# elcritch/figdraw

Measured on AMD Instinct MI355X. Metric: Mpixels/s composited @3840x2160, 300 SDF rects+shadows; % HBM roofline, higher is better.
Workload: dtype f32 (blur taps: u8 x f16 -> f32 MFMA); 1 GPU; S300@4K: renderlist_100 scene at 3840x2160, 300 shadowed SDF rects + full-frame and 360x240 2-pass Gaussian backdrop blur(18) (BASELINE.json configs[2]); draws=707, phases=3, blur_nodes=2, fragments=41088819, parallelism=single GPU, frames_in_flight_per_gpu=4, walk_pool_threads=7, walk_pool_threads_default=7

## Files before the change

### figdraw_amd/csrc/fdh_capi.cpp

```cpp
#include <string>

#include "fdh_context.h"
#include "fdh_damage.h"
#include "../../include/figdraw_hip_damage.h"
#include "../../include/figdraw_hip_pick.h"
#include "../../include/figdraw_hip_readback.h"
#include "../../include/figdraw_hip_stream.h"
#include "../../include/figdraw_hip_exact.h"
#include "../../include_glyphs/figdraw_hip_glyphs.h"
#include "../../include_glyphs/figdraw_hip_coverage.h"
#include "../../include_glyphs/figdraw_hip_cubic.h"

using fdh::Context;

namespace {
thread_local std::string g_last_error;

template <typename F>
int guard(F&& f) {
  try {
    f();
    return FDH_OK;
  } catch (const fdh::Error& e) {
    g_last_error = e.what();
// ... 12 lines not shown
}
}

extern "C" {

const char* fdh_last_error(void) { return g_last_error.c_str(); }
#if FDH_STATS
extern "C++" { namespace fdh { void debug_counters(unsigned long long out[128], bool reset); void debug_wave_times(unsigned long long* out); } }
__attribute__((visibility("default"))) int fdh_debug_wave_times(unsigned long long* out) { fdh::debug_wave_times(out); return 0; }
__attribute__((visibility("default"))) int fdh_debug_counters(unsigned long long out[128], int reset) { fdh::debug_counters(out, reset != 0); return 0; }
#endif
int fdh_saturated_core(const float rect[4], const float rx[4], const float ry[4], int mode, float factor, float spread,
                       const float shape[2], float aa, int out_px[4]) {
  return guard([&] { fdh::saturated_core_of(rect, rx, ry, mode, factor, spread, shape, aa, out_px); });
}
int fdh_blur_weight_fragments(float blur_radius, int vertical, float* dense, uint16_t* frag_bits, int* reach, int* k_steps) {
  return guard([&] {
    if (!dense || !frag_bits || !reach || !k_steps) throw fdh::Error(FDH_ERR_INVALID, "fdh_blur_weight_fragments: null pointer");
    fdh::blur_weight_fragments(blur_radius, vertical != 0, dense, frag_bits, reach, k_steps);
  });
}
const char* fdh_version(void) { return "figdraw_hip 0.1.0 (gfx950)"; }
int fdh_sizeof_fig(void) { return (int)sizeof(FdhFig); }
int fdh_sizeof_glyph(void) { return (int)sizeof(FdhGlyph); }
int fdh_sizeof_draw_op(void) { return (int)sizeof(FdhDrawOp); }
int fdh_sizeof_text_rect(void) { return (int)sizeof(FdhTextRect); }

int fdh_create(FdhContext** out, int atlas_size, float pixel_scale, int device, uint32_t flags) {
  return guard([&] {
    if (!out) throw fdh::Error(FDH_ERR_INVALID, "fdh_create: null out pointer");
// ... 325 lines not shown
```

### figdraw_amd/csrc/fdh_context.h

```cpp
#pragma once
#include <hip/hip_runtime.h>

#include <algorithm>
#include <atomic>
#include <chrono>
#include <condition_variable>
#include <cstdint>
#include <cstdlib>
#include <cstring>
#include <exception>
#include <memory>
#include <mutex>
#include <stdexcept>
#include <string>
#include <thread>
#include <unordered_map>
#include <vector>

#include "../../include/figdraw_hip.h"
#include "../../include/figdraw_hip_pick.h"
#include "../../include/figdraw_hip_readback.h"
#include "../../include/figdraw_hip_stream.h"
#include "fdh_kernels.h"
#include "fdh_plain.h"
#include "fdh_memory.h"
#include "fdh_frame.h"
#include "fdh_atlas.h"
#include "fdh_damage_host.h"
#include "fdh_retained.h"

namespace fdh {

struct RectMaskEntry { int kind; };
class Context;
struct SerialOnly {};

class Recorder {
 public:
  Recorder(Context* cx, bool is_main) : cx_(cx), is_main_(is_main) {}
  void save_transform();
  void restore_transform();
  void translate(float x, float y);
  void rotate(float a);
  void scale(float sx, float sy);
  void apply_transform(const float m[16]);
  bool transform_mirrors_y() const;
  void set_aa(float aa);
  float aa() const { return aa_; }
  void draw_rounded_rect_sdf(const float rect[4], const FdhColor colors[4], const float rx[4], const float ry[4], int mode,
                             float factor, float spread, const float shape[2], int fill_mode, FdhColor mid, FdhColor stop,
// ... 36 lines not shown
  BBox outer_union_{0, 0, 0, 0};
  int depth_now_ = 0;
  PhaseSum sum_;
  int64_t fragments_ = 0, culled_draws_ = 0;
  int phase_floor_ = 0;
  PickTag tag_{-1, -1};

 protected:
  DrawRec& next_rec();
  bool emit_quad(DrawRec& r, float x0, float y0, float x1, float y1, bool count_fragments);
  bool emit_quad_pts(DrawRec& r, const float vx[4], const float vy[4], bool count_fragments);
  struct QuadPx { float px[4], py[4]; BBox b; bool finite; };
  void quad_corners(const float vx[4], const float vy[4], QuadPx& q) const;
  bool emit_corners(DrawRec& r, const QuadPx& q, bool count_fragments);
  void push_rec(BBox b);
  void commit_bins(uint32_t idx);
  void link_share(uint32_t idx);
  bool bbox_visible(const BBox& b) const;
  struct EntryUV { const AtlasEntry* e; float S, x, y, w, h; };
  EntryUV entry_uv(int64_t key) const;
  struct PixelQuad { float x0, y0, x1, y1, w, h; };
  PixelQuad axis_lod(DrawRec& r, float S, float x0, float y0, float x1, float y1) const;
  void rect_entry();
  void white_texel_uv(DrawRec& r) const;
  void shrink_to_ink(const AtlasEntry& e, bool use_alpha, int level_t);
  friend class Context;
};

class Context : public Recorder {
 public:
// ... 277 lines not shown
};

template <typename Buf> void Context::reserve_quiet(Buf& buf, size_t n) {
  if (n <= buf.cap) return;
  drain();
  FDH_HIP(hipStreamSynchronize(stream_));
  buf.reserve(n);
}

void record_host_form(DrawRec& r);
void stripe_rows(int height, int world, int rank, int* y0, int* y1);
void comm_unique_id(uint8_t out[FDH_COMM_ID_BYTES]);
void blur_weight_fragments(float blur_radius, bool vertical, float* dense, uint16_t* frag_bits, int* reach, int* k_steps);
void saturated_core_of(const float rect[4], const float rx[4], const float ry[4], int mode, float factor, float spread,
                       const float shape[2], float aa, int out[4]);

}
```

### figdraw_amd/csrc/fdh_device.h

```cpp
#pragma once
#include <hip/hip_runtime.h>
#include <hip/hip_ext.h>
#include <stdint.h>
#include <algorithm>
#include <type_traits>

#include "fdh_kernels.h"

#include <cstddef>
#include <cstdlib>

namespace fdh {

#ifndef FDH_STATS
#define FDH_STATS 0
#endif
#ifndef FDH_TIMING
#define FDH_TIMING 0
#endif
#ifndef FDH_SPLIT_UNIFORM
#define FDH_SPLIT_UNIFORM 0
#endif
#if FDH_TIMING
#define FDH_NOW() clock64()
// ... 283 lines not shown
  x1 = x1 > kBin ? kBin : x1; y1 = y1 > kBin ? kBin : y1;
  const int r0 = y0 >> 3, r1 = (y1 + 7) >> 3;
  const uint32_t rows = ((1u << r1) - 1u) & ~((1u << r0) - 1u);
  return strips_of_rows(rows, x0 < kTileW, x1 > kTileW);
}

__device__ __forceinline__ uint32_t strip_mask_inside(int x0, int y0, int x1, int y1) {
  int r0 = (y0 + 7) >> 3, r1 = y1 >> 3;
  r0 = r0 < 0 ? 0 : r0; r0 = r0 > 8 ? 8 : r0; r1 = r1 > 8 ? 8 : r1;
  r1 = r1 < r0 ? r0 : r1;
  const uint32_t rows = ((1u << r1) - 1u) & ~((1u << r0) - 1u);
  const uint32_t m = strips_of_rows(rows, x0 <= 0 && x1 >= kTileW, x0 <= kTileW && x1 >= 2 * kTileW);
  return m & (0u - (uint32_t)(x1 > x0 && y1 > y0));
}

__device__ __forceinline__ bool bin_entry_head(const BinRec* __restrict__ binrec, int i, int x0, int y0, BinRec& r, uint32_t& word, uint32_t& strips) {
  {
    const uint2* __restrict__ src = reinterpret_cast<const uint2*>(binrec + i);
    uint2 q0 = src[0], q1 = src[1], q2 = src[2];
    asm volatile("" : "+v"(q0), "+v"(q1), "+v"(q2));
    r.box.x0 = (int16_t)(q0.x & 0xffffu); r.box.y0 = (int16_t)(q0.x >> 16); r.box.x1 = (int16_t)(q0.y & 0xffffu); r.box.y1 = (int16_t)(q0.y >> 16);
    r.ix0 = (int16_t)(q1.x & 0xffffu); r.iy0 = (int16_t)(q1.x >> 16); r.ix1 = (int16_t)(q1.y & 0xffffu); r.iy1 = (int16_t)(q1.y >> 16);
    r.flags = q2.x; r.pad = q2.y;
  }
  const BBox b = r.box;
  strips = strip_mask(b.x0 - x0, b.y0 - y0, b.x1 - x0, b.y1 - y0);
  word = (uint32_t)i | (r.flags & ~LE_INDEX);
  return b.x0 < x0 + kBin && b.x1 > x0 && b.y0 < y0 + kBin && b.y1 > y0;
}
__device__ __forceinline__ void bin_entry_tail(const BinRec& r, int x0, int y0, bool& hit, uint32_t& strips) {
  const uint32_t m_core = 0u - (uint32_t)((r.flags & BR_HAS_CORE) != 0u), m_removed = 0u - (uint32_t)((r.flags & BR_CORE_REMOVED) != 0u),
                 m_exact = 0u - (uint32_t)((r.flags & BR_BOX_EXACT) != 0u);
  const uint32_t core = strip_mask_inside(r.ix0 - x0, r.iy0 - y0, r.ix1 - x0, r.iy1 - y0) & strips & m_core;
  const uint32_t s1 = (strips & ~(core & m_removed)) | ((core & ~m_removed) << 16);
  const uint32_t m_gone = m_core & m_removed & (0u - (uint32_t)((s1 & 0xffffu) == 0u));
  const BBox b = r.box;
  const uint32_t inq = strip_mask_inside(b.x0 - x0, b.y0 - y0, b.x1 - x0, b.y1 - y0) & s1 & ~(s1 >> 16) & 0xffffu & m_core & m_exact & ~m_gone;
  strips = (s1 & ~inq) | (inq << 16);
  hit = hit && m_gone == 0u;
}

struct Frag {
  float u, v;
  F4 col;
  float fw_u, fw_v, lod;
  bool covered;
};

// ... 197 lines not shown
```

### figdraw_amd/csrc/fdh_record.cpp

```cpp
#include <algorithm>
#include <cmath>
#include <cstdio>
#include <cstring>

#include "fdh_context.h"
#include "fdh_host.h"

namespace fdh {

void Recorder::shrink_to_ink(const AtlasEntry& e, bool use_alpha, int level_t) {
  static const bool enabled = [] { const char* v = std::getenv("FDH_INK_BOUNDS"); return !v || std::atoi(v) != 0; }();
  if (!enabled || !e.has_ink || level_t < 0 || lane_->recs.empty()) return;
  DrawRec& r = lane_->recs.back();
  BBox& b = lane_->bins.back().box;
  if ((r.op_mode & F_GENERAL) || b.x1 <= b.x0 || b.y1 <= b.y0) return;
  const InkBox ib = (use_alpha ? e.ink_a : e.ink_rgb)[std::min(level_t / 16, kInkLevels - 1)];
  if (ib.x1 <= ib.x0 || ib.y1 <= ib.y0) { b = BBox{0, 0, 0, 0}; r.bx0 = r.by0 = r.bx1 = r.by1 = 0; return; }
  const double S = (double)cx_->atlas_.size();
  auto range = [&](double ua, double ut, double o, double inv, double lo_t, double hi_t, int& p0, int& p1) {
    const double A = (ut - ua) * inv * S, B = ua * S - 0.5 - A * o;
    if (!(std::fabs(A) > 1e-12)) return;
    double c0 = ((lo_t - 3.0) - B) / A, c1 = ((hi_t + 2.0) - B) / A;
    if (c0 > c1) std::swap(c0, c1);
    if (!(c0 > -1.0e6 && c1 < 1.0e6)) return;
// ... 80 lines not shown
void Recorder::apply_transform(const float m[16]) {
  { FDH_REC("apply_transform").fv(m, 16); }
  Aff n;
  n.a = m[0]; n.b = m[1]; n.c = m[4]; n.d = m[5]; n.tx = m[12]; n.ty = m[13];
  mat_ = aff_mul(mat_, n);
}
bool Recorder::transform_mirrors_y() const { return mat_.a * mat_.d - mat_.b * mat_.c < 0.0f; }

DrawRec& Recorder::next_rec() {
  DrawRec* r = lane_->recs.slot();
  std::memset(static_cast<void*>(r), 0, sizeof *r);
  return *r;
}
void Recorder::push_rec(BBox b) {
  BinRec* br = lane_->bins.slot();
  *br = BinRec{b, 0, 0, 0, 0, 0u, 0u};
  *lane_->boxes.slot() = 0x7f7f7f7fu;
  lane_->recs.n++;
  lane_->bins.n++;
  lane_->boxes.n++;
  if (cx_->pick_frame_) { *lane_->tags.slot() = tag_; lane_->tags.n++; }
}

uint32_t bin_box_of(const BBox& b, int shift) {
  if (bbox_empty(b)) return 0x7f7f7f7fu;
  return (uint32_t)(b.x0 >> shift) | ((uint32_t)(b.y0 >> shift) << 8) | ((127u - (uint32_t)((b.x1 - 1) >> shift)) << 16) | ((127u - (uint32_t)((b.y1 - 1) >> shift)) << 24);
}

static uint32_t binrec_flags(const DrawRec& r) {
  const uint32_t om = r.op_mode, op = (om >> 12) & 15u, mode = om & 255u, fill_mode = (om >> 9) & 7u;
  const bool atlas_mode = mode == 0u || (mode >= 13u && mode <= 16u);
// ... 148 lines not shown
    int run = 0;
    int* row = diff.data() + (size_t)y * dw;
    const int* above = y > ty0 ? row - dw : nullptr;
    for (int x = tx0; x < tx1; x++) {
      run += row[x];
      const int cell = run + (above ? above[x] : 0);
      row[x] = cell;
      mx = std::max(mx, cell);
    }
  }
  for (int y = ty0; y <= ty1; y++) std::fill(diff.begin() + (size_t)y * dw + tx0, diff.begin() + (size_t)y * dw + tx1 + 1, 0);
  touched = false;
  return mx;
}

static bool local_core(const DrawRec& r, double& xl, double& xr, double& yb, double& yt) {
  const uint32_t mode = r.op_mode & 255u, op = (r.op_mode >> 12) & 15u;
  const uint32_t fill_mode = (r.op_mode >> 9) & 7u;
  if (!(op == OP_DRAW || op == OP_MASK_PUSH) || !(r.aa > 0.0f)) return false;
  double e;
  if (op == OP_MASK_PUSH || mode == FDH_SDF_CLIP_AA || mode == FDH_SDF_BACKDROP_BLUR) e = 0.5 / r.aa;
  else if (mode == FDH_SDF_DROP_SHADOW) e = std::max(0.0, -(double)(fill_mode == 0u ? r.f1 : 0.0f));
  else if (mode == FDH_SDF_ANNULAR || mode == FDH_SDF_ANNULAR_AA) e = std::max(0.0, (double)r.f0) + 0.5 / r.aa;
  else if (mode == FDH_SDF_INSET_SHADOW && op == OP_DRAW) {
    const double sigma = std::max(0.5 * (double)r.f0, 0.5);
    e = std::max(0.0, 3.7 * sigma + (double)(fill_mode == 0u ? r.f1 : 0.0f));
  } else return false;
  const bool inset = mode == FDH_SDF_INSET_SHADOW;
  const double qhx = r.p0, qhy = r.p1, bx = inset ? qhx : (double)r.p2, by = inset ? qhy : (double)r.p3;
  if (!(qhx > 0.0 && qhy > 0.0 && bx > 0.0 && by > 0.0)) return false;
  double crx[4], cry[4];
  for (int k = 0; k < 4; k++) {
    const double sel = r.r[k];
    if (!(r.op_mode & F_ELLIP)) { crx[k] = cry[k] = std::max(sel, 0.0); continue; }
    if (sel < 0.0) { crx[k] = cry[k] = -sel - 1.0; continue; }
    const double pv = std::floor(sel + 0.5), hi = std::floor(pv / 4096.0);
    crx[k] = (pv - 4096.0 * hi) * bx / 4095.0;
    cry[k] = hi * by / 4095.0;
  }
  enum { TR = 0, BR = 1, TL = 2, BL = 3 };
  if (!(r.op_mode & F_ELLIP)) {
    const double k = 0.2929;
    auto rr = [&](int i) { return std::max(crx[i] - e, 0.0); };
    xr = (bx - e) - k * std::max(rr(TR), rr(BR));
    xl = -(bx - e) + k * std::max(rr(TL), rr(BL));
    yt = (by - e) - k * std::max(rr(TR), rr(TL));
    yb = -(by - e) + k * std::max(rr(BR), rr(BL));
  } else {
    const double hx0 = -(bx - e), hx1 = bx - e;
    const double hy1 = std::min(by - e, by - std::max(cry[TR], cry[TL])), hy0 = -std::min(by - e, by - std::max(cry[BR], cry[BL]));
    const double vy0 = -(by - e), vy1 = by - e;
    const double vx1 = std::min(bx - e, bx - std::max(crx[TR], crx[BR])), vx0 = -std::min(bx - e, bx - std::max(crx[TL], crx[BL]));
    const double ah = std::max(hx1 - hx0, 0.0) * std::max(hy1 - hy0, 0.0), av = std::max(vx1 - vx0, 0.0) * std::max(vy1 - vy0, 0.0);
    if (ah >= av) { xl = hx0; xr = hx1; yb = hy0; yt = hy1; } else { xl = vx0; xr = vx1; yb = vy0; yt = vy1; }
  }
  if (inset) { xl += r.p2; xr += r.p2; yb -= r.p3; yt -= r.p3; }
  return xr > xl && yt > yb;
}
static void set_saturated_core(DrawRec& r, float w_px, float h_px) {
  r.ix0 = r.iy0 = r.ix1 = r.iy1 = 0;
  double xl, xr, yb, yt;
  if (!local_core(r, xl, xr, yb, yt)) return;
  const double qhx = r.p0, qhy = r.p1;
#ifndef FDH_CORE_SLACK
#define FDH_CORE_SLACK (1.0 / 16.0)
#endif
  const double slack = FDH_CORE_SLACK;
  const double cxl = r.ox + w_px * (xl / (2.0 * qhx) + 0.5) + slack, cxr = r.ox + w_px * (xr / (2.0 * qhx) + 0.5) - slack;
  const double cyt = r.oy + h_px * (0.5 - yt / (2.0 * qhy)) + slack, cyb = r.oy + h_px * (0.5 - yb / (2.0 * qhy)) - slack;
  double ix0 = std::ceil(cxl - 0.5), ix1 = std::floor(cxr - 0.5) + 1.0, iy0 = std::ceil(cyt - 0.5), iy1 = std::floor(cyb - 0.5) + 1.0;
  ix0 = std::max(ix0, (double)r.ox); ix1 = std::min(ix1, (double)r.ox + w_px);
  iy0 = std::max(iy0, (double)r.oy); iy1 = std::min(iy1, (double)r.oy + h_px);
  auto c16 = [](double v) { return (int16_t)std::min(std::max(v, -32768.0), 32767.0); };
  if (!(ix1 > ix0 && iy1 > iy0)) return;
  r.ix0 = c16(ix0); r.iy0 = c16(iy0); r.ix1 = c16(ix1); r.iy1 = c16(iy1);
}

bool Recorder::emit_quad(DrawRec& r, float x0, float y0, float x1, float y1, bool count_fragments) {
  const float vx[4] = {x0, x1, x1, x0}, vy[4] = {y1, y1, y0, y0};
  return emit_quad_pts(r, vx, vy, count_fragments);
}

bool Recorder::rect_visible(const float rect[4], float pad) const {
  if (!(rect[2] > 0.0f) || !(rect[3] > 0.0f)) return false;
  const float vx[4] = {rect[0], rect[0] + rect[2], rect[0] + rect[2], rect[0]}, vy[4] = {rect[1] + rect[3], rect[1] + rect[3], rect[1], rect[1]};
  float minx = 0, maxx = 0, miny = 0, maxy = 0;
  for (int i = 0; i < 4; i++) {
    const float px = std::ceil(mat_.a * vx[i] + mat_.c * vy[i] + mat_.tx), py = std::ceil(mat_.b * vx[i] + mat_.d * vy[i] + mat_.ty);
    if (i == 0) { minx = maxx = px; miny = maxy = py; }
    else { minx = std::min(minx, px); maxx = std::max(maxx, px); miny = std::min(miny, py); maxy = std::max(maxy, py); }
// ... 22 lines not shown
  q.finite = minx > -lim && maxx < lim && miny > -lim && maxy < lim;
  if (!q.finite) return;
  const float W = (float)cx_->W_, H = (float)cx_->H_;
  q.b.x0 = (int16_t)clampf(minx, 0.0f, W); q.b.x1 = (int16_t)clampf(maxx, 0.0f, W);
  q.b.y0 = (int16_t)clampf(miny, 0.0f, H); q.b.y1 = (int16_t)clampf(maxy, 0.0f, H);
}
bool Recorder::emit_quad_pts(DrawRec& r, const float vx[4], const float vy[4], bool count_fragments) {
  QuadPx q;
  quad_corners(vx, vy, q);
  return emit_corners(r, q, count_fragments);
}
bool Recorder::emit_corners(DrawRec& r, const QuadPx& q, bool count_fragments) {
  const float* px = q.px;
  const float* py = q.py;
  BBox b = q.b;
  const bool cullable = ((r.op_mode >> 12) & 15u) == OP_DRAW && culling();
  const float fields[] = {r.p0, r.p1, r.p2, r.p3, r.f0, r.f1, r.r[0], r.r[1], r.r[2], r.r[3], r.aa, r.aux, r.aux2};
  bool params_finite = true;
  for (const float v : fields) params_finite = params_finite && std::isfinite(v);
  if (!q.finite || !params_finite) {
    if (cullable) { FDH_CULLED(); return false; }
    r.bx0 = r.by0 = r.bx1 = r.by1 = 0; push_rec(b); return true;
  }
  if (cullable && !bbox_visible(b)) { FDH_CULLED(); return false; }
  r.bx0 = b.x0; r.by0 = b.y0; r.bx1 = b.x1; r.by1 = b.y1;
  const bool aligned = px[3] == px[0] && px[2] == px[1] && py[3] == py[2] && py[0] == py[1] && px[1] > px[0] && py[0] > py[3];
  const bool bezier = (r.op_mode & 255u) >= 18u && (r.op_mode & 255u) <= 20u;
  if (aligned) {
    r.ox = px[3];
    r.oy = py[3];
    r.inv_w = 1.0f / (px[1] - px[0]);
    r.inv_h = 1.0f / (py[0] - py[3]);
    r.kx = 2.0f * r.p0 * r.inv_w;
    r.ky = 2.0f * r.p1 * r.inv_h;
    if (!bezier) set_saturated_core(r, px[1] - px[0], py[0] - py[3]);
  }
  if (!aligned || bezier) {
    QuadExt& q = *lane_->exts.slot();
    std::memset(static_cast<void*>(&q), 0, sizeof q);
    static const int TRI[2][3] = {{3, 0, 1}, {2, 3, 1}};
    const uint32_t mode = r.op_mode & 255u;
    const bool atlas_mode = mode == 0u || (mode >= 13u && mode <= 16u);
    const float uax = atlas_mode ? r.r[0] : 0.0f, uay = atlas_mode ? r.r[1] : 0.0f, utx = atlas_mode ? r.r[2] : 1.0f, uty = atlas_mode ? r.r[3] : 1.0f;
    const float vu[4] = {uax, utx, utx, uax}, vv[4] = {uty, uty, uay, uay};
    bool edge32 = true;
    const long long xm = 2LL * cx_->W_ + 129, ym = 2LL * cx_->H_ + 129;
    for (int t = 0; t < 2; t++) {
      long long X[3], Y[3];
      for (int k = 0; k < 3; k++) { X[k] = 2 * (long long)px[TRI[t][k]]; Y[k] = 2 * (long long)py[TRI[t][k]]; }
      long long area2 = (X[1] - X[0]) * (Y[2] - Y[0]) - (Y[1] - Y[0]) * (X[2] - X[0]);
// ... 25 lines not shown
        const double dv1 = vv[TRI[t][1]] - vv[TRI[t][0]], dv2 = vv[TRI[t][2]] - vv[TRI[t][0]];
        const double dudx = (du1 * e2y - du2 * e1y) / det, dudy = (du2 * e1x - du1 * e2x) / det;
        const double dvdx = (dv1 * e2y - dv2 * e1y) / det, dvdy = (dv2 * e1x - dv1 * e2x) / det;
        q.fw_u[t] = (float)(std::fabs(dudx) + std::fabs(dudy));
        q.fw_v[t] = (float)(std::fabs(dvdx) + std::fabs(dvdy));
        const double S = (double)cx_->atlas_.size();
        const double rho = std::max(std::sqrt(dudx * dudx + dvdx * dvdx), std::sqrt(dudy * dudy + dvdy * dvdy)) * S;
        q.lod[t] = rho > 0.0 ? (float)std::log2(rho) : 0.0f;
      } else {
        q.fw_u[t] = q.fw_v[t] = 1.0f;
      }
    }
    r.op_mode |= F_GENERAL;
    if (edge32) r.op_mode |= F_EDGE32;
    q.core[0] = q.core[1] = q.core[2] = q.core[3] = 0.0f;
    double xl, xr, yb, yt;
    if (edge32 && !atlas_mode && mode < 18u && ((r.op_mode >> 12) & 15u) == OP_DRAW && q.inv_sum[0] != 0.0f && q.inv_sum[1] != 0.0f && local_core(r, xl, xr, yb, yt)) {
      const double qhx = r.p0, qhy = r.p1;
      double sx = 0.0, sy = 0.0;
      for (int t = 0; t < 2; t++) {
        const QuadExt::Edge &E0 = q.e[t][0], &E1 = q.e[t][1], &E2 = q.e[t][2];
        const double is = (double)q.inv_sum[t];
        const double ua = t == 0 ? (double)E2.a : (double)E0.a + E2.a, ub = t == 0 ? (double)E2.b : (double)E0.b + E2.b, uc = t == 0 ? (double)E2.c : (double)E0.c + (double)E2.c;
        const double va = t == 0 ? (double)E1.a + E2.a : (double)E2.a, vb = t == 0 ? (double)E1.b + E2.b : (double)E2.b, vc = t == 0 ? (double)E1.c + (double)E2.c : (double)E2.c;
        const double kx = 2.0 * qhx * is, ky = -2.0 * qhy * is;
        const double m[6] = {kx * ua, kx * ub, kx * uc - qhx, ky * va, ky * vb, ky * vc + qhy};
        for (int k = 0; k < 6; k++) q.lm[t][k] = (float)m[k];
        sx = std::max(sx, 2.0 * (std::fabs(m[0]) + std::fabs(m[1])));
        sy = std::max(sy, 2.0 * (std::fabs(m[3]) + std::fabs(m[4])));
      }
#ifndef FDH_CORE_SLACK
#define FDH_CORE_SLACK (1.0 / 16.0)
// ... 61 lines not shown

void saturated_core_of(const float rect[4], const float rx[4], const float ry[4], int mode, float factor, float spread,
                       const float shape[2], float aa, int out[4]) {
  const FdhColor white{255, 255, 255, 255}, zero{0, 0, 0, 0};
  const FdhColor cols[4] = {white, white, white, white};
  DrawRec r;
  std::memset(static_cast<void*>(&r), 0, sizeof r);
  fill_sdf_rec(r, rect, cols, rx, ry, mode, factor, spread, shape, 0, zero, zero, 0.5f, aa);
  const float x0 = std::ceil(rect[0]), y0 = std::ceil(rect[1]), x1 = std::ceil(rect[0] + rect[2]), y1 = std::ceil(rect[1] + rect[3]);
  out[0] = out[1] = out[2] = out[3] = 0;
  if (!(x1 > x0 && y1 > y0)) return;
  r.ox = x0; r.oy = y0;
  r.inv_w = 1.0f / (x1 - x0); r.inv_h = 1.0f / (y1 - y0);
  set_saturated_core(r, x1 - x0, y1 - y0);
  out[0] = r.ix0; out[1] = r.iy0; out[2] = r.ix1; out[3] = r.iy1;
}

void Recorder::draw_rounded_rect_sdf(const float rect[4], const FdhColor colors[4], const float rx[4], const float ry[4], int mode,
                                    float factor, float spread, const float shape[2], int fill_mode, FdhColor mid, FdhColor stop,
                                    float mid_pos) {
  { FDH_REC("draw_rounded_rect_sdf").fv(rect, 4).cols(colors).fv(rx, 4).fv(ry, 4).i(mode).f(factor).f(spread).fv(shape, 2).i(fill_mode).col(mid).col(stop).f(mid_pos); }
  if (!cx_->frame_begun_) throw Error(FDH_ERR_INVALID, "ctx.beginFrame has not been called.");
  if (!(rect[2] > 0.0f) || !(rect[3] > 0.0f)) return;
  if (mode >= FDH_SDF_BEZIER_STROKE_AA) throw Error(FDH_ERR_INVALID, "bezier stroke modes go through drawQuadraticBezierSdf");
  QuadPx q;
  {
    const float x0 = rect[0], y0 = rect[1], x1 = rect[0] + rect[2], y1 = rect[1] + rect[3];
    const float vx[4] = {x0, x1, x1, x0}, vy[4] = {y1, y1, y0, y0};
    quad_corners(vx, vy, q);
  }
// ... 452 lines not shown
```

### figdraw_amd/csrc/fdh_types.h

```cpp
#pragma once
#include <stdint.h>

#ifndef FDH_MX_LO
#define FDH_MX_LO 0
#endif

namespace fdh {

constexpr int kTile = 8;
constexpr int kTileW = 4 * kTile;
constexpr int kTileH = kTile;
constexpr int kWavesPerWg = 4;
constexpr int kWgW = kTileW;
constexpr int kWgH = kTileH * kWavesPerWg;
constexpr int kBin = 64;
constexpr int kWgsPerBin = (kBin / kWgW) * (kBin / kWgH);
constexpr int kMaskDepth = 16;
constexpr int kDeepMinDefault = 24;
constexpr int kDeepMinInFlight = 40;
constexpr int kDeepStripMinDefault = 16;
constexpr int kMaxMips = 14;
constexpr int kMaxBlurTaps = 36;

enum : uint32_t { OP_DRAW = 0, OP_MASK_PUSH = 1, OP_MASK_POP = 2, OP_RMASK_BEGIN = 3, OP_RMASK_END = 4 };
// ... 30 lines not shown
struct alignas(16) QuadExt {
  struct Edge { int32_t a, b; int64_t c; };
  Edge e[2][3];
  float inv_sum[2];
  uint32_t own;
  float fw_u[2], fw_v[2];
  float lod[2];
  float _pad[3];
  float core[4];
  float lm[2][6];
};
static_assert(sizeof(QuadExt) == 208 && offsetof(QuadExt, core) == 144 && offsetof(QuadExt, lm) == 160, "QuadExt: 208 bytes, core at 144, lm at 160");

struct alignas(8) BBox { int16_t x0, y0, x1, y1; };

struct alignas(8) BinRec { BBox box; int16_t ix0, iy0, ix1, iy1; uint32_t flags; uint32_t pad; };
static_assert(sizeof(BinRec) == 24, "BinRec must be 24 bytes");
constexpr uint32_t BR_HAS_CORE = 1u, BR_CORE_REMOVED = 2u;
constexpr uint32_t BR_GENERAL = 4u;
constexpr uint32_t BR_CURVE = 8u;
constexpr uint32_t BR_BOX_EXACT = 16u;
constexpr uint32_t LE_PLAIN = 1u << 31;
constexpr uint32_t LE_OPAQUE = 1u << 30;
constexpr int LE_PATH_SHIFT = 26;
constexpr uint32_t LE_SHARE = 1u << 25;
constexpr uint32_t LE_INDEX = LE_SHARE - 1u;

constexpr int kMaxBlurReach = 66;
constexpr int kBlurPad = 15;
struct BlurTaps {
  int n;
  int reach;
// ... 23 lines not shown
```

### figdraw_amd/csrc/k_bin_upload.hip

```cpp
#include "fdh_device.h"

namespace fdh {
__device__ __forceinline__ bool binbox_hits(uint32_t q, uint32_t U) { return ((U - q) & 0x80808080u) == 0x80808080u; }
template <bool kRefine>
__device__ __forceinline__ void bin_entry(const BinParams& P, int i, int x0, int y0, bool& hit, uint32_t& word, uint32_t& strips) {
  BinRec r;
  if (!bin_entry_head(P.binrec, i, x0, y0, r, word, strips)) { hit = false; return; }
  if (kRefine && (r.flags & BR_CURVE)) {
    const uint4* __restrict__ d4 = reinterpret_cast<const uint4*>(P.draws + i);
    const uint4 q0 = d4[0], q1 = d4[1], q2 = d4[2], q3 = d4[3], q5 = d4[5];
    const float ox = __uint_as_float(q0.z), oy = __uint_as_float(q0.w), inv_w = __uint_as_float(q1.x), inv_h = __uint_as_float(q1.y);
    const float p0 = __uint_as_float(q1.z), p1 = __uint_as_float(q1.w), Ax = __uint_as_float(q2.x), Ay = __uint_as_float(q2.y), f0 = __uint_as_float(q2.z);
    const float Bx = __uint_as_float(q3.x), By = __uint_as_float(q3.y), Cx = __uint_as_float(q3.z), Cy = __uint_as_float(q3.w), aa = __uint_as_float(q5.z);
    CurveBox cb[2];
    curve_boxes2(Ax, Ay, Bx, By, Cx, Cy, cb);
    const float reach = 1.41422f * (__builtin_fmaxf(f0, 0.0f) * 0.5f + 0.5f / aa) + 0.05f;
    const float sx = inv_w * (2.0f * p0), sy = inv_h * (2.0f * p1);
    const float tx = (-ox * inv_w - 0.5f) * (2.0f * p0), ty = (-oy * inv_h - 0.5f) * (2.0f * p1);
    const float asx = __builtin_fabsf(sx), asy = __builtin_fabsf(sy);
    float X0[2], Y0[2], dXc[2], dXr[2], dYc[2], dYr[2], ex[2], ey[2], bcx[2], bcy[2];
    bool bin_near = false;
    const float eps = 0.002f;
#pragma unroll
    for (int c = 0; c < 2; c++) {
// ... 205 lines not shown

__global__ __launch_bounds__(64) void k_upload_frame(uint8_t* __restrict__ dst, UploadTable T) {
  const uint32_t lane = threadIdx.x;
  const UploadRun R = T.run[blockIdx.y];
  const uint32_t at = blockIdx.x * 1024u;
  if (at >= R.bytes) return;
  if (R.kind == 1u) {
    const uint32_t ush = 6u + T.binbox_shift;
#pragma unroll
    for (int h = 0; h < 2; h++) {
      const uint32_t o = at + (lane + 64u * h) * 8u;
      if (o >= R.bytes) continue;
      const uint2 v = *reinterpret_cast<const uint2*>(static_cast<const uint8_t*>(R.src) + o);
      *reinterpret_cast<uint2*>(dst + R.dst_off + o) = v;
      const uint32_t rel = R.dst_off - T.bins_off + o;
      if (rel % 24u != 0u) continue;
      const uint32_t draw = rel / 24u;
      const int x0 = (int)(int16_t)(v.x & 0xffffu), y0 = (int)(int16_t)(v.x >> 16), x1 = (int)(int16_t)(v.y & 0xffffu), y1 = (int)(int16_t)(v.y >> 16);
      uint32_t q = 0x7f7f7f7fu;
      if (x1 > x0 && y1 > y0)
        q = (uint32_t)(x0 >> ush) | ((uint32_t)(y0 >> ush) << 8) | ((127u - (uint32_t)((x1 - 1) >> ush)) << 16) | ((127u - (uint32_t)((y1 - 1) >> ush)) << 24);
      uint32_t* box = reinterpret_cast<uint32_t*>(dst + T.box_off);
      box[draw] = q;
      if (draw + 1u == T.n_draws)
        for (uint32_t k = draw + 1u; (k & 3u) != 0u; k++) box[k] = 0x7f7f7f7fu;
    }
    return;
  }
  const uint32_t o = at + lane * 16u;
  if (o >= R.bytes) return;
  uint4 v = *reinterpret_cast<const uint4*>(static_cast<const uint8_t*>(R.src) + o);
  if (R.kind == 2u && (o & 127u) == 0u && (v.x & F_GENERAL)) v.y += R.ext_add;
// ... 18 lines not shown
```

### figdraw_amd/csrc/k_composite_strip.inc

```
  static_assert(kRole == 0 || (kPaths == 4 && kFull), "deep strips: the no-clip build's full-frame launch only");
  constexpr int kStripsPerBin = kWgsPerBin * kWavesPerWg;
  constexpr int mslot = 0;
  constexpr bool kBlender = kRole == 1, kShader = kRole == 2;
  constexpr bool kOpaque = (kPaths & 32) != 0;
  static_assert(!kOpaque || (kPaths == (4 | 32) && kRole == 0), "the opaque form exists for the no-clip build only");
  using FT = std::conditional_t<kOpaque, F4o, F4>;
  uint32_t (*mask_stack)[kMaskDepth][64] = reinterpret_cast<uint32_t (*)[kMaskDepth][64]>(composite_lds);
  const DeepRing ring(composite_lds);
  uint32_t rank = 0, unit = 0;
  const int tx1 = tx0 + kTileW, ty1 = ty0 + kTileH;
  const int px0 = tx0 + (lane & 7) * 4, py = ty0 + (lane >> 3);
  const size_t spill_at = ((size_t)bin * kStripsPerBin + (size_t)sidx) * 64 + (size_t)lane;
  auto stack_put = [&](const int depth, const uint32_t v) __attribute__((always_inline)) {
    if (depth < kMaskDepth) mask_stack[mslot][depth][lane] = v;
    else __hip_atomic_store(P.mask_spill + (size_t)(depth - kMaskDepth) * P.spill_stride + spill_at, v, __ATOMIC_RELAXED, __HIP_MEMORY_SCOPE_AGENT);
  };
  auto stack_get = [&](const int depth) __attribute__((always_inline)) -> uint32_t {
    if (depth < kMaskDepth) return mask_stack[mslot][depth][lane];
    return __hip_atomic_load(P.mask_spill + (size_t)(depth - kMaskDepth) * P.spill_stride + spill_at, __ATOMIC_RELAXED, __HIP_MEMORY_SCOPE_AGENT);
  };
  constexpr bool kMasks = (kPaths & 4) == 0;
#if FDH_TIMING
  const unsigned long long T0 = FDH_NOW(), W0 = wall_clock64();
  unsigned long long T_cull = 0, T_rec = 0, T_shade = 0, T_cnt = 0, n_draws_t = 0, T_cull_core = 0, n_core_t = 0, n_all_t = 0;
// ... 91 lines not shown
      const float ia = __uint_as_float(__builtin_amdgcn_readfirstlane(h5));
      blend_pre(F0, c_rg, c_ba, ia); blend_pre(F1, c_rg, c_ba, ia); blend_pre(F2, c_rg, c_ba, ia); blend_pre(F3, c_rg, c_ba, ia);
    }
    __hip_atomic_store(ring.consumed, rk + 1u, __ATOMIC_RELEASE, __HIP_MEMORY_SCOPE_WORKGROUP);
  };
  for (uint32_t base = 0; base < cnt; base += 64) {
#if FDH_TIMING
    const unsigned long long Tc0 = FDH_NOW();
#endif
    const uint32_t i = base + lane;
    uint2 e;
    if (direct) {
      const int by = bin / P.bins_x, bx = bin - by * P.bins_x;
      BinRec br;
      uint32_t word = 0, strips = 0;
      bool hit = bin_entry_head(P.binrec, P.direct_first + (int)min(i, cnt - 1u), bx * kBin, by * kBin, br, word, strips);
      bin_entry_tail(br, bx * kBin, by * kBin, hit, strips);
      e = make_uint2(word, hit ? strips : 0u);
    } else {
      e = list[min(i, cnt - 1u)];
    }
    const uint32_t idx = e.x;
    const uint32_t ey = i < cnt ? e.y : 0u;
    const uint32_t st = (ey >> sbit) & 0x10001u;
    unsigned long long m = __ballot(st != 0u);
    const unsigned long long m_core = __ballot(st == 0x10001u);
    const unsigned long long m_inq = __ballot(st == 0x10000u);
    if (!kMasks || !P.has_masks) {
      const unsigned long long m_opaque = __ballot(st == 0x10001u && (idx & LE_OPAQUE) != 0u);
      if (m_opaque != 0) m &= ~((1ull << (63 - __builtin_clzll(m_opaque))) - 1ull);
    }
#if FDH_TIMING
// ... 1171 lines not shown
```

Baseline: 192,400 Mpixels/s.

## Extend saturated-core culling to a union of core plus horizontal/vertical bands

The host now computes, besides the main inscribed saturated core of each rounded rect, a horizontal and a vertical band rectangle, and packs their offsets into a BinRec grown from 24 to 32 bytes. The binning tail ORs the band strip masks into the core mask, so more strips get classified as fully covered, and occluded draws underneath can be skipped. The direct composite path keeps the old single-core test. The cost is a larger BinRec (more upload and load bandwidth), an extra 8-byte load per entry, and more host work per draw. An env var controls it, on by default.

```diff
diff --git a/figdraw_amd/csrc/fdh_capi.cpp b/figdraw_amd/csrc/fdh_capi.cpp
--- a/figdraw_amd/csrc/fdh_capi.cpp
+++ b/figdraw_amd/csrc/fdh_capi.cpp
@@ -50,6 +50,13 @@
                        const float shape[2], float aa, int out_px[4]) {
   return guard([&] { fdh::saturated_core_of(rect, rx, ry, mode, factor, spread, shape, aa, out_px); });
 }
+__attribute__((visibility("default"))) int fdh_saturated_core_union(const float rect[4], const float rx[4], const float ry[4], int mode, float factor, float spread,
+                             const float shape[2], float aa, int push, int out_px[12], int* n_out) {
+  return guard([&] {
+    if (!out_px || !n_out) throw fdh::Error(FDH_ERR_INVALID, "fdh_saturated_core_union: null pointer");
+    *n_out = fdh::saturated_core_union_of(rect, rx, ry, mode, factor, spread, shape, aa, push, out_px);
+  });
+}
 int fdh_blur_weight_fragments(float blur_radius, int vertical, float* dense, uint16_t* frag_bits, int* reach, int* k_steps) {
   return guard([&] {
     if (!dense || !frag_bits || !reach || !k_steps) throw fdh::Error(FDH_ERR_INVALID, "fdh_blur_weight_fragments: null pointer");
diff --git a/figdraw_amd/csrc/fdh_context.h b/figdraw_amd/csrc/fdh_context.h
--- a/figdraw_amd/csrc/fdh_context.h
+++ b/figdraw_amd/csrc/fdh_context.h
@@ -34,6 +34,8 @@
 struct RectMaskEntry { int kind; };
 class Context;
 struct SerialOnly {};
+
+struct CoreBands { uint32_t grow = 0; uint16_t hy0 = 0, hy1 = 0, vx0 = 0, vx1 = 0; };
 
 class Recorder {
  public:
@@ -100,6 +102,7 @@
   void quad_corners(const float vx[4], const float vy[4], QuadPx& q) const;
   bool emit_corners(DrawRec& r, const QuadPx& q, bool count_fragments);
   void push_rec(BBox b);
+  CoreBands bands_;
   void commit_bins(uint32_t idx);
   void link_share(uint32_t idx);
   bool bbox_visible(const BBox& b) const;
@@ -407,5 +410,8 @@
 void blur_weight_fragments(float blur_radius, bool vertical, float* dense, uint16_t* frag_bits, int* reach, int* k_steps);
 void saturated_core_of(const float rect[4], const float rx[4], const float ry[4], int mode, float factor, float spread,
                        const float shape[2], float aa, int out[4]);
+int saturated_core_union_of(const float rect[4], const float rx[4], const float ry[4], int mode, float factor, float spread,
+                            const float shape[2], float aa, int push, int out[12]);
+int binrec_core_rects(const BinRec& br, int out[12]);
 
 }
diff --git a/figdraw_amd/csrc/fdh_device.h b/figdraw_amd/csrc/fdh_device.h
--- a/figdraw_amd/csrc/fdh_device.h
+++ b/figdraw_amd/csrc/fdh_device.h
@@ -321,24 +321,36 @@
   return m & (0u - (uint32_t)(x1 > x0 && y1 > y0));
 }
 
+template <bool kUnion = true>
 __device__ __forceinline__ bool bin_entry_head(const BinRec* __restrict__ binrec, int i, int x0, int y0, BinRec& r, uint32_t& word, uint32_t& strips) {
   {
     const uint2* __restrict__ src = reinterpret_cast<const uint2*>(binrec + i);
-    uint2 q0 = src[0], q1 = src[1], q2 = src[2];
-    asm volatile("" : "+v"(q0), "+v"(q1), "+v"(q2));
+    uint2 q0 = src[0], q1 = src[1], q2 = src[2], q3 = make_uint2(0u, 0u);
+    if (kUnion) {
+      q3 = src[3];
+      asm volatile("" : "+v"(q0), "+v"(q1), "+v"(q2), "+v"(q3));
+    } else {
+      asm volatile("" : "+v"(q0), "+v"(q1), "+v"(q2));
+    }
     r.box.x0 = (int16_t)(q0.x & 0xffffu); r.box.y0 = (int16_t)(q0.x >> 16); r.box.x1 = (int16_t)(q0.y & 0xffffu); r.box.y1 = (int16_t)(q0.y >> 16);
     r.ix0 = (int16_t)(q1.x & 0xffffu); r.iy0 = (int16_t)(q1.x >> 16); r.ix1 = (int16_t)(q1.y & 0xffffu); r.iy1 = (int16_t)(q1.y >> 16);
-    r.flags = q2.x; r.pad = q2.y;
+    r.flags = q2.x; r.grow = q2.y;
+    r.hy0 = (uint16_t)(q3.x & 0xffffu); r.hy1 = (uint16_t)(q3.x >> 16); r.vx0 = (uint16_t)(q3.y & 0xffffu); r.vx1 = (uint16_t)(q3.y >> 16);
   }
   const BBox b = r.box;
   strips = strip_mask(b.x0 - x0, b.y0 - y0, b.x1 - x0, b.y1 - y0);
   word = (uint32_t)i | (r.flags & ~LE_INDEX);
   return b.x0 < x0 + kBin && b.x1 > x0 && b.y0 < y0 + kBin && b.y1 > y0;
 }
+template <bool kUnion = true>
 __device__ __forceinline__ void bin_entry_tail(const BinRec& r, int x0, int y0, bool& hit, uint32_t& strips) {
   const uint32_t m_core = 0u - (uint32_t)((r.flags & BR_HAS_CORE) != 0u), m_removed = 0u - (uint32_t)((r.flags & BR_CORE_REMOVED) != 0u),
                  m_exact = 0u - (uint32_t)((r.flags & BR_BOX_EXACT) != 0u);
-  const uint32_t core = strip_mask_inside(r.ix0 - x0, r.iy0 - y0, r.ix1 - x0, r.iy1 - y0) & strips & m_core;
+  const int cx0 = r.ix0 - x0, cy0 = r.iy0 - y0, cx1 = r.ix1 - x0, cy1 = r.iy1 - y0;
+  const int gx0 = (int)(r.grow & 255u), gx1 = (int)((r.grow >> 8) & 255u), gy0 = (int)((r.grow >> 16) & 255u), gy1 = (int)(r.grow >> 24);
+  uint32_t in_core = strip_mask_inside(cx0, cy0, cx1, cy1);
+  if (kUnion) in_core |= strip_mask_inside(cx0 - gx0, cy0 + (int)r.hy0, cx1 + gx1, cy1 - (int)r.hy1) | strip_mask_inside(cx0 + (int)r.vx0, cy0 - gy0, cx1 - (int)r.vx1, cy1 + gy1);
+  const uint32_t core = in_core & strips & m_core;
   const uint32_t s1 = (strips & ~(core & m_removed)) | ((core & ~m_removed) << 16);
   const uint32_t m_gone = m_core & m_removed & (0u - (uint32_t)((s1 & 0xffffu) == 0u));
   const BBox b = r.box;
diff --git a/figdraw_amd/csrc/fdh_record.cpp b/figdraw_amd/csrc/fdh_record.cpp
--- a/figdraw_amd/csrc/fdh_record.cpp
+++ b/figdraw_amd/csrc/fdh_record.cpp
@@ -118,7 +118,8 @@
 }
 void Recorder::push_rec(BBox b) {
   BinRec* br = lane_->bins.slot();
-  *br = BinRec{b, 0, 0, 0, 0, 0u, 0u};
+  *br = BinRec{b, 0, 0, 0, 0, 0u, bands_.grow, bands_.hy0, bands_.hy1, bands_.vx0, bands_.vx1};
+  bands_ = CoreBands{};
   *lane_->boxes.slot() = 0x7f7f7f7fu;
   lane_->recs.n++;
   lane_->bins.n++;
@@ -297,7 +298,11 @@
   return mx;
 }
 
-static bool local_core(const DrawRec& r, double& xl, double& xr, double& yb, double& yt) {
+struct LocalRect {
+  double xl, xr, yb, yt;
+  bool ok() const { return xr > xl && yt > yb; }
+};
+static bool local_core(const DrawRec& r, LocalRect out[3]) {
   const uint32_t mode = r.op_mode & 255u, op = (r.op_mode >> 12) & 15u;
   const uint32_t fill_mode = (r.op_mode >> 9) & 7u;
   if (!(op == OP_DRAW || op == OP_MASK_PUSH) || !(r.aa > 0.0f)) return false;
@@ -322,41 +327,87 @@
     cry[k] = hi * by / 4095.0;
   }
   enum { TR = 0, BR = 1, TL = 2, BL = 3 };
+  LocalRect &H = out[1], &V = out[2];
+  H.xl = -(bx - e); H.xr = bx - e;
+  V.yb = -(by - e); V.yt = by - e;
   if (!(r.op_mode & F_ELLIP)) {
     const double k = 0.2929;
     auto rr = [&](int i) { return std::max(crx[i] - e, 0.0); };
-    xr = (bx - e) - k * std::max(rr(TR), rr(BR));
-    xl = -(bx - e) + k * std::max(rr(TL), rr(BL));
-    yt = (by - e) - k * std::max(rr(TR), rr(TL));
-    yb = -(by - e) + k * std::max(rr(BR), rr(BL));
+    const double mr = std::max(rr(TR), rr(BR)), ml = std::max(rr(TL), rr(BL)), mt = std::max(rr(TR), rr(TL)), mb = std::max(rr(BR), rr(BL));
+    out[0].xr = (bx - e) - k * mr;
+    out[0].xl = -(bx - e) + k * ml;
+    out[0].yt = (by - e) - k * mt;
+    out[0].yb = -(by - e) + k * mb;
+    H.yt = (by - e) - mt; H.yb = -(by - e) + mb;
+    V.xr = (bx - e) - mr; V.xl = -(bx - e) + ml;
   } else {
-    const double hx0 = -(bx - e), hx1 = bx - e;
-    const double hy1 = std::min(by - e, by - std::max(cry[TR], cry[TL])), hy0 = -std::min(by - e, by - std::max(cry[BR], cry[BL]));
-    const double vy0 = -(by - e), vy1 = by - e;
-    const double vx1 = std::min(bx - e, bx - std::max(crx[TR], crx[BR])), vx0 = -std::min(bx - e, bx - std::max(crx[TL], crx[BL]));
-    const double ah = std::max(hx1 - hx0, 0.0) * std::max(hy1 - hy0, 0.0), av = std::max(vx1 - vx0, 0.0) * std::max(vy1 - vy0, 0.0);
-    if (ah >= av) { xl = hx0; xr = hx1; yb = hy0; yt = hy1; } else { xl = vx0; xr = vx1; yb = vy0; yt = vy1; }
-  }
-  if (inset) { xl += r.p2; xr += r.p2; yb -= r.p3; yt -= r.p3; }
-  return xr > xl && yt > yb;
-}
-static void set_saturated_core(DrawRec& r, float w_px, float h_px) {
-  r.ix0 = r.iy0 = r.ix1 = r.iy1 = 0;
-  double xl, xr, yb, yt;
-  if (!local_core(r, xl, xr, yb, yt)) return;
+    H.yt = std::min(by - e, by - std::max(cry[TR], cry[TL])); H.yb = -std::min(by - e, by - std::max(cry[BR], cry[BL]));
+    V.xr = std::min(bx - e, bx - std::max(crx[TR], crx[BR])); V.xl = -std::min(bx - e, bx - std::max(crx[TL], crx[BL]));
+    const double ah = std::max(H.xr - H.xl, 0.0) * std::max(H.yt - H.yb, 0.0), av = std::max(V.xr - V.xl, 0.0) * std::max(V.yt - V.yb, 0.0);
+    out[0] = ah >= av ? H : V;
+  }
+  if (inset)
+    for (int k = 0; k < 3; k++) { out[k].xl += r.p2; out[k].xr += r.p2; out[k].yb -= r.p3; out[k].yt -= r.p3; }
+  return true;
+}
+static bool core_pixels(const DrawRec& r, float w_px, float h_px, const LocalRect& c, int16_t px[4]) {
+  if (!c.ok()) return false;
   const double qhx = r.p0, qhy = r.p1;
 #ifndef FDH_CORE_SLACK
 #define FDH_CORE_SLACK (1.0 / 16.0)
 #endif
   const double slack = FDH_CORE_SLACK;
-  const double cxl = r.ox + w_px * (xl / (2.0 * qhx) + 0.5) + slack, cxr = r.ox + w_px * (xr / (2.0 * qhx) + 0.5) - slack;
-  const double cyt = r.oy + h_px * (0.5 - yt / (2.0 * qhy)) + slack, cyb = r.oy + h_px * (0.5 - yb / (2.0 * qhy)) - slack;
+  const double cxl = r.ox + w_px * (c.xl / (2.0 * qhx) + 0.5) + slack, cxr = r.ox + w_px * (c.xr / (2.0 * qhx) + 0.5) - slack;
+  const double cyt = r.oy + h_px * (0.5 - c.yt / (2.0 * qhy)) + slack, cyb = r.oy + h_px * (0.5 - c.yb / (2.0 * qhy)) - slack;
   double ix0 = std::ceil(cxl - 0.5), ix1 = std::floor(cxr - 0.5) + 1.0, iy0 = std::ceil(cyt - 0.5), iy1 = std::floor(cyb - 0.5) + 1.0;
   ix0 = std::max(ix0, (double)r.ox); ix1 = std::min(ix1, (double)r.ox + w_px);
   iy0 = std::max(iy0, (double)r.oy); iy1 = std::min(iy1, (double)r.oy + h_px);
   auto c16 = [](double v) { return (int16_t)std::min(std::max(v, -32768.0), 32767.0); };
-  if (!(ix1 > ix0 && iy1 > iy0)) return;
-  r.ix0 = c16(ix0); r.iy0 = c16(iy0); r.ix1 = c16(ix1); r.iy1 = c16(iy1);
+  if (!(ix1 > ix0 && iy1 > iy0)) return false;
+  px[0] = c16(ix0); px[1] = c16(iy0); px[2] = c16(ix1); px[3] = c16(iy1);
+  return true;
+}
+static bool core_union_on() {
+  static const bool enabled = [] { const char* v = std::getenv("FDH_CORE_UNION"); return !v || std::atoi(v) != 0; }();
+  return enabled;
+}
+static CoreBands pack_bands(const int16_t c[4], const int16_t* h, const int16_t* v) {
+  CoreBands b;
+  auto u8 = [](int d) { return (uint32_t)std::min(d, 255); };
+  auto u16 = [](int d) { return (uint16_t)std::min(d, 65535); };
+  if (h && h[0] <= c[0] && h[2] >= c[2] && h[1] >= c[1] && h[3] <= c[3]) {
+    b.grow |= u8(c[0] - h[0]) | (u8(h[2] - c[2]) << 8);
+    b.hy0 = u16(h[1] - c[1]); b.hy1 = u16(c[3] - h[3]);
+  }
+  if (v && v[1] <= c[1] && v[3] >= c[3] && v[0] >= c[0] && v[2] <= c[2]) {
+    b.grow |= (u8(c[1] - v[1]) << 16) | (u8(v[3] - c[3]) << 24);
+    b.vx0 = u16(v[0] - c[0]); b.vx1 = u16(c[2] - v[2]);
+  }
+  return b;
+}
+int binrec_core_rects(const BinRec& br, int out[12]) {
+  const int g[4] = {(int)(br.grow & 255u), (int)((br.grow >> 8) & 255u), (int)((br.grow >> 16) & 255u), (int)(br.grow >> 24)};
+  const int q[3][4] = {{br.ix0, br.iy0, br.ix1, br.iy1},
+                       {br.ix0 - g[0], br.iy0 + (int)br.hy0, br.ix1 + g[1], br.iy1 - (int)br.hy1},
+                       {br.ix0 + (int)br.vx0, br.iy0 - g[2], br.ix1 - (int)br.vx1, br.iy1 + g[3]}};
+  int n = 0;
+  for (int k = 0; k < 3; k++) {
+    const bool ok = q[k][2] > q[k][0] && q[k][3] > q[k][1];
+    for (int j = 0; j < 4; j++) out[4 * k + j] = ok ? q[k][j] : 0;
+    n += ok ? 1 : 0;
+  }
+  return n;
+}
+static CoreBands set_saturated_core(DrawRec& r, float w_px, float h_px) {
+  r.ix0 = r.iy0 = r.ix1 = r.iy1 = 0;
+  LocalRect lc[3];
+  if (!local_core(r, lc)) return CoreBands{};
+  int16_t c[4], h[4], v[4];
+  if (!core_pixels(r, w_px, h_px, lc[0], c)) return CoreBands{};
+  r.ix0 = c[0]; r.iy0 = c[1]; r.ix1 = c[2]; r.iy1 = c[3];
+  if (!core_union_on()) return CoreBands{};
+  const bool hok = core_pixels(r, w_px, h_px, lc[1], h), vok = core_pixels(r, w_px, h_px, lc[2], v);
+  return pack_bands(c, hok ? h : nullptr, vok ? v : nullptr);
 }
 
 bool Recorder::emit_quad(DrawRec& r, float x0, float y0, float x1, float y1, bool count_fragments) {
@@ -409,6 +460,7 @@
   const float* px = q.px;
   const float* py = q.py;
   BBox b = q.b;
+  bands_ = CoreBands{};
   const bool cullable = ((r.op_mode >> 12) & 15u) == OP_DRAW && culling();
   const float fields[] = {r.p0, r.p1, r.p2, r.p3, r.f0, r.f1, r.r[0], r.r[1], r.r[2], r.r[3], r.aa, r.aux, r.aux2};
   bool params_finite = true;
@@ -428,7 +480,7 @@
     r.inv_h = 1.0f / (py[0] - py[3]);
     r.kx = 2.0f * r.p0 * r.inv_w;
     r.ky = 2.0f * r.p1 * r.inv_h;
-    if (!bezier) set_saturated_core(r, px[1] - px[0], py[0] - py[3]);
+    if (!bezier) bands_ = set_saturated_core(r, px[1] - px[0], py[0] - py[3]);
   }
   if (!aligned || bezier) {
     QuadExt& q = *lane_->exts.slot();
@@ -484,8 +536,9 @@
     r.op_mode |= F_GENERAL;
     if (edge32) r.op_mode |= F_EDGE32;
     q.core[0] = q.core[1] = q.core[2] = q.core[3] = 0.0f;
-    double xl, xr, yb, yt;
-    if (edge32 && !atlas_mode && mode < 18u && ((r.op_mode >> 12) & 15u) == OP_DRAW && q.inv_sum[0] != 0.0f && q.inv_sum[1] != 0.0f && local_core(r, xl, xr, yb, yt)) {
+    LocalRect lc[3];
+    if (edge32 && !atlas_mode && mode < 18u && ((r.op_mode >> 12) & 15u) == OP_DRAW && q.inv_sum[0] != 0.0f && q.inv_sum[1] != 0.0f && local_core(r, lc) && lc[0].ok()) {
+      double xl = lc[0].xl, xr = lc[0].xr, yb = lc[0].yb, yt = lc[0].yt;
       const double qhx = r.p0, qhy = r.p1;
       double sx = 0.0, sy = 0.0;
       for (int t = 0; t < 2; t++) {
@@ -577,6 +630,23 @@
   r.inv_w = 1.0f / (x1 - x0); r.inv_h = 1.0f / (y1 - y0);
   set_saturated_core(r, x1 - x0, y1 - y0);
   out[0] = r.ix0; out[1] = r.iy0; out[2] = r.ix1; out[3] = r.iy1;
+}
+int saturated_core_union_of(const float rect[4], const float rx[4], const float ry[4], int mode, float factor, float spread,
+                            const float shape[2], float aa, int push, int out[12]) {
+  const FdhColor white{255, 255, 255, 255}, zero{0, 0, 0, 0};
+  const FdhColor cols[4] = {white, white, white, white};
+  DrawRec r;
+  std::memset(static_cast<void*>(&r), 0, sizeof r);
+  fill_sdf_rec(r, rect, cols, rx, ry, mode, factor, spread, shape, 0, zero, zero, 0.5f, aa);
+  if (push) r.op_mode |= OP_MASK_PUSH << 12;
+  const float x0 = std::ceil(rect[0]), y0 = std::ceil(rect[1]), x1 = std::ceil(rect[0] + rect[2]), y1 = std::ceil(rect[1] + rect[3]);
+  for (int k = 0; k < 12; k++) out[k] = 0;
+  if (!(x1 > x0 && y1 > y0)) return 0;
+  r.ox = x0; r.oy = y0;
+  r.inv_w = 1.0f / (x1 - x0); r.inv_h = 1.0f / (y1 - y0);
+  const CoreBands b = set_saturated_core(r, x1 - x0, y1 - y0);
+  const BinRec br{BBox{0, 0, 0, 0}, r.ix0, r.iy0, r.ix1, r.iy1, 0u, b.grow, b.hy0, b.hy1, b.vx0, b.vx1};
+  return binrec_core_rects(br, out);
 }
 
 void Recorder::draw_rounded_rect_sdf(const float rect[4], const FdhColor colors[4], const float rx[4], const float ry[4], int mode,
diff --git a/figdraw_amd/csrc/fdh_types.h b/figdraw_amd/csrc/fdh_types.h
--- a/figdraw_amd/csrc/fdh_types.h
+++ b/figdraw_amd/csrc/fdh_types.h
@@ -68,8 +68,8 @@
 
 struct alignas(8) BBox { int16_t x0, y0, x1, y1; };
 
-struct alignas(8) BinRec { BBox box; int16_t ix0, iy0, ix1, iy1; uint32_t flags; uint32_t pad; };
-static_assert(sizeof(BinRec) == 24, "BinRec must be 24 bytes");
+struct alignas(8) BinRec { BBox box; int16_t ix0, iy0, ix1, iy1; uint32_t flags; uint32_t grow; uint16_t hy0, hy1, vx0, vx1; };
+static_assert(sizeof(BinRec) == 32, "BinRec must be 32 bytes");
 constexpr uint32_t BR_HAS_CORE = 1u, BR_CORE_REMOVED = 2u;
 constexpr uint32_t BR_GENERAL = 4u;
 constexpr uint32_t BR_CURVE = 8u;
diff --git a/figdraw_amd/csrc/k_bin_upload.hip b/figdraw_amd/csrc/k_bin_upload.hip
--- a/figdraw_amd/csrc/k_bin_upload.hip
+++ b/figdraw_amd/csrc/k_bin_upload.hip
@@ -243,8 +243,8 @@
       const uint2 v = *reinterpret_cast<const uint2*>(static_cast<const uint8_t*>(R.src) + o);
       *reinterpret_cast<uint2*>(dst + R.dst_off + o) = v;
       const uint32_t rel = R.dst_off - T.bins_off + o;
-      if (rel % 24u != 0u) continue;
-      const uint32_t draw = rel / 24u;
+      if (rel % (uint32_t)sizeof(BinRec) != 0u) continue;
+      const uint32_t draw = rel / (uint32_t)sizeof(BinRec);
       const int x0 = (int)(int16_t)(v.x & 0xffffu), y0 = (int)(int16_t)(v.x >> 16), x1 = (int)(int16_t)(v.y & 0xffffu), y1 = (int)(int16_t)(v.y >> 16);
       uint32_t q = 0x7f7f7f7fu;
       if (x1 > x0 && y1 > y0)
diff --git a/figdraw_amd/csrc/k_composite_strip.inc b/figdraw_amd/csrc/k_composite_strip.inc
--- a/figdraw_amd/csrc/k_composite_strip.inc
+++ b/figdraw_amd/csrc/k_composite_strip.inc
@@ -129,8 +129,8 @@
       const int by = bin / P.bins_x, bx = bin - by * P.bins_x;
       BinRec br;
       uint32_t word = 0, strips = 0;
-      bool hit = bin_entry_head(P.binrec, P.direct_first + (int)min(i, cnt - 1u), bx * kBin, by * kBin, br, word, strips);
-      bin_entry_tail(br, bx * kBin, by * kBin, hit, strips);
+      bool hit = bin_entry_head<false>(P.binrec, P.direct_first + (int)min(i, cnt - 1u), bx * kBin, by * kBin, br, word, strips);
+      bin_entry_tail<false>(br, bx * kBin, by * kBin, hit, strips);
       e = make_uint2(word, hit ? strips : 0u);
     } else {
       e = list[min(i, cnt - 1u)];
```

After: 194,500 Mpixels/s, median of 6. 1.1% higher.
